# canyagmur/XPoint

Hardware: AMD Instinct MI355X
Metric: image-pairs/sec (detect+describe+match) 480x640 optical-thermal (higher is better)
Workload: dtype f32 (dense layers: f32 operands as 2 fp16 terms (operand error <= 2^-23, dropped cross term <= 2^-22: per product <= 2^-21 worst case, ~2^-25 typical), 3 fp16-MFMA partial products, f32 accumulate — GEMMs, implicit-GEMM convolutions and the fused block kernels alike; the deep-stage scan's dt project

## Files before the change

### xpoint_amd/csrc/elementwise.hip

```cpp
#include <stdlib.h>

#include <string>

#include <algorithm>

#include "glue_core.h"

namespace {

__global__ __launch_bounds__(256) void layernorm_kernel(const float* __restrict__ x, float* __restrict__ y,
                                                        const float* __restrict__ w, const float* __restrict__ b,
                                                        int64_t M, int C, float eps, int gelu) {
    const int lane = threadIdx.x & 63;
    const int64_t row = (int64_t)blockIdx.x * 4 + (threadIdx.x >> 6);
    if (row >= M) return;
    const float* xr = x + row * C;
    float v[16];
    float s = 0.f;
#pragma unroll
    for (int i = 0; i < 16; ++i) {
        const int c = lane + 64 * i;
        v[i] = (c < C) ? xr[c] : 0.f;
        s += v[i];
    }
// ... 13 lines not shown
        if (c < C) {
            float o = (v[i] - mean) * rstd * w[c] + b[c];
            if (gelu) o = xp_gelu(o);
            yr[c] = o;
        }
    }
}

template <int LPR, int NV, int RPG = 1, bool P32 = false>
__global__ __launch_bounds__(256) void layernorm_vec_kernel(const float* __restrict__ x, float* __restrict__ y,
                                                            const float* __restrict__ w, const float* __restrict__ b,
                                                            int64_t M, int C, float eps, int gelu) {
    constexpr int RPW = 64 / LPR;
    const int lane = threadIdx.x & 63, sub = lane % LPR;
    const int64_t row0 = ((int64_t)blockIdx.x * 4 + (threadIdx.x >> 6)) * (RPW * RPG) + lane / LPR;
    const int C4 = C >> 2;
    float4 v[RPG][NV];
    bool rok[RPG];
#pragma unroll
    for (int r = 0; r < RPG; ++r) {
        const int64_t row = row0 + r * RPW;
        rok[r] = row < M;
        const float4* xr = reinterpret_cast<const float4*>(x + (rok[r] ? row : 0) * C);
#pragma unroll
        for (int i = 0; i < NV; ++i) {
            const int c4 = sub + i * LPR;
            v[r][i] = (c4 < C4) ? xr[c4] : make_float4(0.f, 0.f, 0.f, 0.f);
        }
    }
#pragma unroll
    for (int r = 0; r < RPG; ++r) {
        float s = 0.f;
#pragma unroll
        for (int i = 0; i < NV; ++i) s += (v[r][i].x + v[r][i].y) + (v[r][i].z + v[r][i].w);
#pragma unroll
        for (int o = LPR / 2; o > 0; o >>= 1) s += __shfl_xor(s, o, 64);
        const float mean = s / (float)C;
        float q = 0.f;
#pragma unroll
        for (int i = 0; i < NV; ++i) {
            if (sub + i * LPR < C4) {
                const float dx = v[r][i].x - mean, dy = v[r][i].y - mean, dz = v[r][i].z - mean, dw = v[r][i].w - mean;
                q = fmaf(dx, dx, q); q = fmaf(dy, dy, q); q = fmaf(dz, dz, q); q = fmaf(dw, dw, q);
            }
        }
#pragma unroll
        for (int o = LPR / 2; o > 0; o >>= 1) q += __shfl_xor(q, o, 64);
        const float rstd = 1.f / sqrtf(q / (float)C + eps);
        if (!rok[r]) continue;
        float4* yr = reinterpret_cast<float4*>(y + (row0 + r * RPW) * C);
#pragma unroll
        for (int i = 0; i < NV; ++i) {
            const int c4 = sub + i * LPR;
            if (c4 < C4) {
                const float4 wv = reinterpret_cast<const float4*>(w)[c4], bv = reinterpret_cast<const float4*>(b)[c4];
                float4 o;
                o.x = (v[r][i].x - mean) * rstd * wv.x + bv.x; o.y = (v[r][i].y - mean) * rstd * wv.y + bv.y;
                o.z = (v[r][i].z - mean) * rstd * wv.z + bv.z; o.w = (v[r][i].w - mean) * rstd * wv.w + bv.w;
                if (gelu) { o.x = xp_gelu(o.x); o.y = xp_gelu(o.y); o.z = xp_gelu(o.z); o.w = xp_gelu(o.w); }
                if (P32) {
                    const xp_h4 hi = {(_Float16)o.x, (_Float16)o.y, (_Float16)o.z, (_Float16)o.w};
                    const xp_h4 lo = {(_Float16)(o.x - (float)hi[0]), (_Float16)(o.y - (float)hi[1]), (_Float16)(o.z - (float)hi[2]), (_Float16)(o.w - (float)hi[3])};
                    const int c = c4 * 4;
                    unsigned char* op = reinterpret_cast<unsigned char*>(y) + ((row0 + r * RPW) * (C >> 5) + (c >> 5)) * 128 + (c & 31) * 2;
                    *reinterpret_cast<xp_h4*>(op) = hi;
                    *reinterpret_cast<xp_h4*>(op + 64) = lo;
                } else
                yr[c4] = o;
            }
        }
    }
}

#ifndef XP_DW_PW
#define XP_DW_PW 4
#endif
#ifndef XP_DW_PH
#define XP_DW_PH 4
#endif
constexpr int DW_PW = XP_DW_PW, DW_PH = XP_DW_PH;
template <bool AMP>
__global__ __launch_bounds__(256) void dwconv3x3_silu_kernel(const float* __restrict__ x, const float* __restrict__ w,
                                                             float* __restrict__ y, int B, int H, int W, int C) {
    xp_dwconv3x3_silu_body<float, AMP, false, DW_PH, DW_PW>(x, w, y, nullptr, B, H, W, C, blockDim.x);
}

template <int CO, bool AMP>
__global__ __launch_bounds__(64) void stem_conv_ln_gelu_kernel(const float* __restrict__ img, const float* __restrict__ w9,
                                                               const float* __restrict__ bias, const float* __restrict__ lnw,
                                                               const float* __restrict__ lnb, float* __restrict__ y,
                                                               int B, int H, int W, float eps) {
    xp_stem_conv_ln_gelu_body<CO, float, AMP>(img, w9, bias, lnw, lnb, y, B, H, W, eps);
}

template <int CO>
__global__ __launch_bounds__(64) void stem_conv_kernel(const float* __restrict__ img, const float* __restrict__ w9, const float* __restrict__ bias,
                                                       float* __restrict__ y, int B, int H, int W) {
    xp_stem_conv_body<CO>(img, w9, bias, y, B, H, W);
}

__global__ __launch_bounds__(256) void depth_to_space_kernel(const float* __restrict__ x, float* __restrict__ y,
                                                             int B, int H, int W, int C, int bs, float limit, int* __restrict__ status) {
    const int Cq = C / (bs * bs);
    const int64_t total = (int64_t)B * H * W * C;
    const int64_t idx = (int64_t)blockIdx.x * blockDim.x + threadIdx.x;
    if (status) {
        const bool bad = idx < total && !(fabsf(x[idx]) < limit);
        if (__ballot(bad) != 0ull && (threadIdx.x & 63) == 0) atomicOr(status, XP_STATUS_ENC);
    }
    if (idx >= total) return;
    const int ch = (int)(idx % C);
    const int64_t pix = idx / C;
    const int w = (int)(pix % W), h = (int)((pix / W) % H);
    const int64_t n = pix / ((int64_t)W * H);
    const int blk = ch / Cq, c = ch - blk * Cq;
    const int i = blk / bs, j = blk - i * bs;
    y[((n * (H * bs) + (h * bs + i)) * (int64_t)(W * bs) + (w * bs + j)) * Cq + c] = x[idx];
}

__global__ __launch_bounds__(256) void depth_to_space_vec_kernel(const float4* __restrict__ x, float4* __restrict__ y,
                                                                 int B, int H, int W, int C4, int bs, float limit, int* __restrict__ status) {
    xp_depth_to_space_vec_body<float>(x, y, nullptr, B, H, W, C4, bs, limit, status, blockDim.x);
}

constexpr int SMX_CPW = 4;
__global__ __launch_bounds__(256) void softmax_shuffle_kernel(const float* __restrict__ logits, float* __restrict__ prob,
                                                              int B, int Hc, int Wc, int r, int ld, int mode, int* __restrict__ status) {
    const int lane = threadIdx.x & 63;
    const int64_t cell0 = ((int64_t)blockIdx.x * 4 + (threadIdx.x >> 6)) * SMX_CPW;
    const int64_t ncell = (int64_t)B * Hc * Wc;
    if (cell0 >= ncell) return;
    const int nch = r * r + 1;
    float v0[SMX_CPW], v1[SMX_CPW];
#pragma unroll
    for (int q = 0; q < SMX_CPW; ++q) {
        const int64_t cell = cell0 + q < ncell ? cell0 + q : ncell - 1;
        const float* lp = logits + cell * ld;
        v0[q] = (lane < nch) ? lp[lane] : -INFINITY;
        v1[q] = (lane + 64 < nch) ? lp[lane + 64] : -INFINITY;
    }
#pragma unroll
    for (int q = 0; q < SMX_CPW; ++q) {
        const int64_t cell = cell0 + q;
        if (cell >= ncell) break;
        float e0, e1, inv;
        if (mode == 0) {
            const float mx = xp_wave_max(fmaxf(v0[q], v1[q]));
            e0 = (lane < nch) ? expf(v0[q] - mx) : 0.f;
            e1 = (lane + 64 < nch) ? expf(v1[q] - mx) : 0.f;
            inv = 1.f / xp_wave_sum(e0 + e1);
            e0 *= inv; e1 *= inv;
            if (status && !(inv <= 1.f) && lane == 0) atomicOr(status, XP_STATUS_PROB);
        } else {
            e0 = (lane < nch) ? expf(v0[q]) : 0.f;
            e1 = (lane + 64 < nch) ? expf(v1[q]) : 0.f;
            const float den = xp_wave_sum(e0 + e1) + 0.00001f;
            e0 = e0 / den; e1 = e1 / den;
        }
        const int w = (int)(cell % Wc), h = (int)((cell / Wc) % Hc);
        const int64_t b = cell / ((int64_t)Wc * Hc);
        const int64_t Wf = (int64_t)Wc * r;
        for (int k = 0; k < 2; ++k) {
            const int ch = lane + 64 * k;
            if (ch < r * r) {
                const int i = ch / r, j = ch - i * r;
                prob[(b * Hc * r + (h * r + i)) * Wf + (w * r + j)] = k ? e1 : e0;
            }
        }
    }
}

// ... 82 lines not shown
    XP_CHECK_ARG(x && y && n >= 0, "xp_round_f16: bad args");
    XP_CHECK_ARG((((uintptr_t)x | (uintptr_t)y) & 15) == 0, "xp_round_f16: buffers must be 16-byte aligned");
    if (n == 0) return XP_OK;
    XpProfScope prof("round_f16", (hipStream_t)stream, 0.0, 8.0 * n);
    hipLaunchKernelGGL(round_f16_kernel, dim3(xp_cdiv(n, 1024)), dim3(256), 0, (hipStream_t)stream, x, y, n);
    XP_LAUNCH_CHECK();
    return XP_OK;
}

static int layernorm_impl(const float* x, float* y, const float* w, const float* b, int64_t rows, int C, float eps, int gelu, void* stream);
extern "C" int xp_layernorm(const float* x, float* y, const float* w, const float* b, int64_t rows, int C, float eps,
                            int gelu, void* stream) {
    if (xp_amp_value()) {
        XP_CHECK_ARG(gelu == 0, "xp_layernorm: the fused GELU has no mixed-precision form (the LayerNorm -> GELU boundary would not be rounded); use xp_stem_conv_ln_gelu or gelu = 0");
        XP_CHECK_ARG(C % 4 == 0 && ((uintptr_t)y & 15) == 0, "xp_layernorm: mixed-precision mode needs C %% 4 == 0 and a 16-byte aligned output (C = %d)", C);
    }
    const int rc = layernorm_impl(x, y, w, b, rows, C, eps, gelu, stream);
    if (rc == XP_OK && xp_amp_value() && rows > 0) return xp_round_f16(y, y, rows * C, stream);
    return rc;
}
static int layernorm_impl(const float* x, float* y, const float* w, const float* b, int64_t rows, int C, float eps,
                          int gelu, void* stream) {
    XP_CHECK_ARG(x && y && w && b, "xp_layernorm: null pointer");
    XP_CHECK_ARG(C > 0 && C <= 1024, "xp_layernorm: C must be in [1,1024] (got %d)", C);
    if (rows == 0) return XP_OK;
    XpProfScope prof(xp_prof_by_shape() ? ("layernorm_C" + std::to_string(C)).c_str() : "layernorm", (hipStream_t)stream, 8.0 * rows * C, 8.0 * rows * C);
    hipStream_t s = (hipStream_t)stream;
    const bool vec = (C % 4 == 0) && ((((uintptr_t)x | (uintptr_t)y | (uintptr_t)w | (uintptr_t)b) & 15) == 0);
    const int C4 = C / 4;
#define XP_LN_LAUNCH(LPR, NV) hipLaunchKernelGGL((layernorm_vec_kernel<LPR, NV, (NV == 1 ? 4 : 1)>), dim3(xp_cdiv(rows, 4 * (64 / LPR) * (NV == 1 ? 4 : 1))), dim3(256), 0, s, x, y, w, b, rows, C, eps, gelu)
    if (!vec) hipLaunchKernelGGL(layernorm_kernel, dim3(xp_cdiv(rows, 4)), dim3(256), 0, s, x, y, w, b, rows, C, eps, gelu);
    else if (C4 <= 4) XP_LN_LAUNCH(4, 1);
    else if (C4 <= 8) XP_LN_LAUNCH(8, 1);
    else if (C4 <= 16) XP_LN_LAUNCH(16, 1);
    else if (C4 <= 32) XP_LN_LAUNCH(32, 1);
    else if (C4 <= 64) XP_LN_LAUNCH(64, 1);
    else if (C4 <= 128) XP_LN_LAUNCH(64, 2);
    else if (C4 <= 192) XP_LN_LAUNCH(64, 3);
    else XP_LN_LAUNCH(64, 4);
#undef XP_LN_LAUNCH
    XP_LAUNCH_CHECK();
    return XP_OK;
}

extern "C" int xp_layernorm_p32(const float* x, void* y_p32, const float* w, const float* b, int64_t rows, int C, float eps, void* stream) {
    XP_CHECK_ARG(x && y_p32 && w && b, "xp_layernorm_p32: null pointer");
    XP_CHECK_ARG(C >= 32 && C <= 1024 && C % 32 == 0, "xp_layernorm_p32: C must be a multiple of 32 in [32, 1024] (got %d)", C);
    XP_CHECK_ARG((((uintptr_t)x | (uintptr_t)y_p32 | (uintptr_t)w | (uintptr_t)b) & 15) == 0, "xp_layernorm_p32: buffers must be 16-byte aligned");
    XP_CHECK_ARG(!xp_amp_value(), "xp_layernorm_p32: no mixed-precision form (the P32 image feeds the f32-grade ring GEMM only)");
    if (rows == 0) return XP_OK;
    XpProfScope prof("layernorm_p32", (hipStream_t)stream, 8.0 * rows * C, 8.0 * rows * C);
    hipStream_t s = (hipStream_t)stream;
    float* y = reinterpret_cast<float*>(y_p32);
    const int C4 = C / 4;
#define XP_LNP_LAUNCH(LPR, NV) hipLaunchKernelGGL((layernorm_vec_kernel<LPR, NV, (NV == 1 ? 4 : 1), true>), dim3(xp_cdiv(rows, 4 * (64 / LPR) * (NV == 1 ? 4 : 1))), dim3(256), 0, s, x, y, w, b, rows, C, eps, 0)
    if (C4 <= 8) XP_LNP_LAUNCH(8, 1);
    else if (C4 <= 16) XP_LNP_LAUNCH(16, 1);
    else if (C4 <= 32) XP_LNP_LAUNCH(32, 1);
    else if (C4 <= 64) XP_LNP_LAUNCH(64, 1);
    else if (C4 <= 128) XP_LNP_LAUNCH(64, 2);
    else if (C4 <= 192) XP_LNP_LAUNCH(64, 3);
    else XP_LNP_LAUNCH(64, 4);
#undef XP_LNP_LAUNCH
    XP_LAUNCH_CHECK();
    return XP_OK;
}

extern "C" int xp_dwconv3x3_silu(const float* x, const float* w9c, float* y, int batch, int H, int W, int C, void* stream) {
    XP_CHECK_ARG(x && w9c && y, "xp_dwconv3x3_silu: null pointer");
    XP_CHECK_ARG(C % 4 == 0, "xp_dwconv3x3_silu: C %% 4 != 0");
    const int64_t total = (int64_t)batch * ((H + DW_PH - 1) / DW_PH) * ((W + DW_PW - 1) / DW_PW) * (C / 4);
    XpProfScope prof("dwconv3x3_silu", (hipStream_t)stream, 22.0 * batch * H * W * C, 8.0 * batch * H * W * C);
    if (xp_amp_value()) hipLaunchKernelGGL(dwconv3x3_silu_kernel<true>, dim3(xp_cdiv(total, 256)), dim3(256), 0, (hipStream_t)stream, x, w9c, y, batch, H, W, C);
    else hipLaunchKernelGGL(dwconv3x3_silu_kernel<false>, dim3(xp_cdiv(total, 256)), dim3(256), 0, (hipStream_t)stream, x, w9c, y, batch, H, W, C);
    XP_LAUNCH_CHECK();
    return XP_OK;
}

extern "C" int xp_stem_conv_ln_gelu(const float* img, const float* w9co, const float* bias, const float* ln_w,
                                    const float* ln_b, float* y, int batch, int H, int W, int Co, float eps, void* stream) {
    XP_CHECK_ARG(img && w9co && bias && ln_w && ln_b && y, "xp_stem_conv_ln_gelu: null pointer");
    const int Ho = H / 2 + (H & 1), Wo = W / 2 + (W & 1);
    const int64_t total = (int64_t)batch * Ho * Wo;
    dim3 grid(xp_cdiv(total, 64)), block(64);
    hipStream_t s = (hipStream_t)stream;
    XpProfScope prof("stem_conv_ln_gelu", (hipStream_t)stream, (double)total * Co * 30.0, 4.0 * ((double)batch * H * W + (double)total * Co));
    const bool amp = xp_amp_value() != 0;
    if (Co == 48 && amp) hipLaunchKernelGGL((stem_conv_ln_gelu_kernel<48, true>), grid, block, 0, s, img, w9co, bias, ln_w, ln_b, y, batch, H, W, eps);
    else if (Co == 16 && amp) hipLaunchKernelGGL((stem_conv_ln_gelu_kernel<16, true>), grid, block, 0, s, img, w9co, bias, ln_w, ln_b, y, batch, H, W, eps);
    else if (Co == 48) hipLaunchKernelGGL((stem_conv_ln_gelu_kernel<48, false>), grid, block, 0, s, img, w9co, bias, ln_w, ln_b, y, batch, H, W, eps);
    else if (Co == 16) hipLaunchKernelGGL((stem_conv_ln_gelu_kernel<16, false>), grid, block, 0, s, img, w9co, bias, ln_w, ln_b, y, batch, H, W, eps);
    else { xp_set_error("xp_stem_conv_ln_gelu: Co must be 48 or 16 (EMBED_DIM 96 / 32), got %d", Co); return XP_ERR_ARG; }
    XP_LAUNCH_CHECK();
    return XP_OK;
}

extern "C" int xp_stem_conv(const float* img, const float* w9co, const float* bias, float* y, int batch, int H, int W, int Co, void* stream) {
    XP_CHECK_ARG(img && w9co && bias && y, "xp_stem_conv: null pointer");
    XP_CHECK_ARG(batch > 0 && H >= 1 && W >= 1, "xp_stem_conv: bad shape batch=%d H=%d W=%d", batch, H, W);
    const int Ho = H / 2 + (H & 1), Wo = W / 2 + (W & 1);
    const int64_t total = (int64_t)batch * Ho * Wo;
    dim3 grid(xp_cdiv(total, 64)), block(64);
    hipStream_t s = (hipStream_t)stream;
    XpProfScope prof("stem_conv", s, (double)total * Co * 18.0, 4.0 * ((double)batch * H * W + (double)total * Co));
    if (Co == 48) hipLaunchKernelGGL(stem_conv_kernel<48>, grid, block, 0, s, img, w9co, bias, y, batch, H, W);
    else if (Co == 16) hipLaunchKernelGGL(stem_conv_kernel<16>, grid, block, 0, s, img, w9co, bias, y, batch, H, W);
    else { xp_set_error("xp_stem_conv: Co must be 48 or 16 (EMBED_DIM 96 / 32), got %d", Co); return XP_ERR_ARG; }
    XP_LAUNCH_CHECK();
    return XP_OK;
}

int xp_depth_to_space_nhwc_st(const float* x, float* y, int batch, int H, int W, int C, int bs, float limit, int* status, void* stream) {
    XP_CHECK_ARG(x && y && C % (bs * bs) == 0, "xp_depth_to_space_nhwc: bad args");
    const int64_t total = (int64_t)batch * H * W * C;
    XpProfScope prof("depth_to_space", (hipStream_t)stream, 0.0, 8.0 * total);
    const bool vec = (C / (bs * bs)) % 4 == 0 && total < (1ll << 31) && ((((uintptr_t)x | (uintptr_t)y) & 15) == 0);
    if (vec) hipLaunchKernelGGL(depth_to_space_vec_kernel, dim3(xp_cdiv(total / 4, 256)), dim3(256), 0, (hipStream_t)stream, reinterpret_cast<const float4*>(x),
                                reinterpret_cast<float4*>(y), batch, H, W, C / 4, bs, limit, status);
    else hipLaunchKernelGGL(depth_to_space_kernel, dim3(xp_cdiv(total, 256)), dim3(256), 0, (hipStream_t)stream, x, y, batch, H, W, C, bs, limit, status);
    XP_LAUNCH_CHECK();
    return XP_OK;
}
extern "C" int xp_depth_to_space_nhwc(const float* x, float* y, int batch, int H, int W, int C, int bs, void* stream) {
    return xp_depth_to_space_nhwc_st(x, y, batch, H, W, C, bs, 0.f, nullptr, stream);
}

extern "C" int xp_softmax_shuffle(const float* logits, float* prob, int batch, int Hc, int Wc, int r, int ld, int mode, void* stream) {
    return xp_softmax_shuffle_st(logits, prob, batch, Hc, Wc, r, ld, mode, nullptr, stream);
}
int xp_softmax_shuffle_st(const float* logits, float* prob, int batch, int Hc, int Wc, int r, int ld, int mode, int* status, void* stream) {
    XP_CHECK_ARG(logits && prob, "xp_softmax_shuffle: null pointer");
    XP_CHECK_ARG(r * r + 1 <= 128 && ld >= r * r + 1, "xp_softmax_shuffle: r*r+1 must be <= 128 and <= ld");
    const int64_t cells = (int64_t)batch * Hc * Wc;
    XpProfScope prof("softmax_shuffle", (hipStream_t)stream, (double)cells * 4.0 * (r * r + 1), 4.0 * cells * (2.0 * r * r + 1));
    hipLaunchKernelGGL(softmax_shuffle_kernel, dim3(xp_cdiv(cells, 4 * SMX_CPW)), dim3(256), 0, (hipStream_t)stream, logits, prob, batch, Hc, Wc, r, ld, mode, status);
    XP_LAUNCH_CHECK();
    return XP_OK;
}

extern "C" int xp_l2norm_rows(const float* x, float* y, int64_t rows, int C, float eps, void* stream) {
    return xp_l2norm_rows_st(x, y, rows, C, eps, nullptr, stream);
}
int xp_l2norm_rows_st(const float* x, float* y, int64_t rows, int C, float eps, int* status, void* stream) {
    XP_CHECK_ARG(x && y, "xp_l2norm_rows: null pointer");
    if (rows == 0) return XP_OK;
    XpProfScope prof("l2norm_rows", (hipStream_t)stream, 3.0 * rows * C, 8.0 * rows * C);
    hipLaunchKernelGGL(l2norm_rows_kernel, dim3(xp_cdiv(rows, 4)), dim3(256), 0, (hipStream_t)stream, x, y, rows, C, eps, status);
    XP_LAUNCH_CHECK();
    return XP_OK;
}

extern "C" int xp_nhwc_to_nchw(const float* x, float* y, int batch, int HW, int C, void* stream) {
    XP_CHECK_ARG(x && y, "xp_nhwc_to_nchw: null pointer");
    dim3 grid(xp_cdiv(HW, 32), xp_cdiv(C, 32), batch);
    XpProfScope prof("nhwc_to_nchw", (hipStream_t)stream, 0.0, 8.0 * batch * HW * C);
    hipLaunchKernelGGL(nhwc_to_nchw_kernel, grid, dim3(256), 0, (hipStream_t)stream, x, y, HW, C);
    XP_LAUNCH_CHECK();
    return XP_OK;
}

__global__ __launch_bounds__(256) void stage_pair_batch_kernel(const float* __restrict__ a, const float* __restrict__ b, float* __restrict__ out,
                                                               const uint8_t* __restrict__ ma, const uint8_t* __restrict__ mb, uint8_t* __restrict__ mout,
                                                               int64_t n) {
    const int64_t stride = (int64_t)gridDim.x * blockDim.x, t0 = (int64_t)blockIdx.x * blockDim.x + threadIdx.x;
    const int64_t n4 = n >> 2;
    const bool al = ((reinterpret_cast<uintptr_t>(a) | reinterpret_cast<uintptr_t>(b) | reinterpret_cast<uintptr_t>(out) | (uintptr_t)(n * 4)) & 15) == 0;
    if (al) {
// ... 147 lines not shown
```

### xpoint_amd/csrc/elementwise_f16.hip

```cpp
#include <stdlib.h>

#include <string>

#include "glue_core.h"
#include "xpoint_hip.h"

namespace {

template <int CO>
__global__ __launch_bounds__(64) void stem_f16_kernel(const float* __restrict__ img, const float* __restrict__ w9, const float* __restrict__ bias,
                                                      const float* __restrict__ lnw, const float* __restrict__ lnb, _Float16* __restrict__ y,
                                                      int B, int H, int W, float eps) {
    xp_stem_conv_ln_gelu_body<CO, _Float16, true>(img, w9, bias, lnw, lnb, y, B, H, W, eps);
}

template <int LPR, int NV>
__global__ __launch_bounds__(256) void layernorm_f16_kernel(const _Float16* __restrict__ x, _Float16* __restrict__ y, const float* __restrict__ w,
                                                            const float* __restrict__ b, int64_t M, int C, float eps) {
    constexpr int RPW = 64 / LPR;
    const int lane = threadIdx.x & 63, sub = lane % LPR;
    const int64_t row = ((int64_t)blockIdx.x * 4 + (threadIdx.x >> 6)) * RPW + lane / LPR;
    const int C8 = C >> 3;
    const bool rok = row < M;
    const xp_h8* xr = reinterpret_cast<const xp_h8*>(x + (rok ? row : 0) * C);
    float v[NV][8];
    float s = 0.f;
#pragma unroll
    for (int i = 0; i < NV; ++i) {
        const int c8 = sub + i * LPR;
        xp_h8 t = {};
        if (c8 < C8) t = xr[c8];
#pragma unroll
        for (int e = 0; e < 8; ++e) { v[i][e] = (float)t[e]; }
        s += ((v[i][0] + v[i][1]) + (v[i][2] + v[i][3])) + ((v[i][4] + v[i][5]) + (v[i][6] + v[i][7]));
    }
#pragma unroll
    for (int o = LPR / 2; o > 0; o >>= 1) s += __shfl_xor(s, o, 64);
    const float mean = s / (float)C;
    float q = 0.f;
#pragma unroll
    for (int i = 0; i < NV; ++i)
        if (sub + i * LPR < C8) {
#pragma unroll
            for (int e = 0; e < 8; ++e) { const float d = v[i][e] - mean; q = fmaf(d, d, q); }
        }
#pragma unroll
    for (int o = LPR / 2; o > 0; o >>= 1) q += __shfl_xor(q, o, 64);
    const float rstd = 1.f / sqrtf(q / (float)C + eps);
    if (!rok) return;
    xp_h8* yr = reinterpret_cast<xp_h8*>(y + row * C);
#pragma unroll
    for (int i = 0; i < NV; ++i) {
        const int c8 = sub + i * LPR;
        if (c8 < C8) {
            const float4 w0 = reinterpret_cast<const float4*>(w)[2 * c8], w1 = reinterpret_cast<const float4*>(w)[2 * c8 + 1];
            const float4 b0 = reinterpret_cast<const float4*>(b)[2 * c8], b1 = reinterpret_cast<const float4*>(b)[2 * c8 + 1];
            const float wv[8] = {w0.x, w0.y, w0.z, w0.w, w1.x, w1.y, w1.z, w1.w}, bv[8] = {b0.x, b0.y, b0.z, b0.w, b1.x, b1.y, b1.z, b1.w};
            xp_h8 o;
#pragma unroll
            for (int e = 0; e < 8; ++e) o[e] = (_Float16)((v[i][e] - mean) * rstd * wv[e] + bv[e]);
            yr[c8] = o;
        }
    }
}

#ifndef XP_DWH_PW
#define XP_DWH_PW 4
#endif
#ifndef XP_DWH_PH
#define XP_DWH_PH 4
#endif
constexpr int DWH_PW = XP_DWH_PW, DWH_PH = XP_DWH_PH;
template <bool F32COPY>
__global__ __launch_bounds__(256) void dwconv3x3_silu_f16_kernel(const _Float16* __restrict__ x, const float* __restrict__ w, _Float16* __restrict__ y,
                                                                 float* __restrict__ y32, int B, int H, int W, int C) {
    xp_dwconv3x3_silu_body<_Float16, true, F32COPY, DWH_PH, DWH_PW>(x, w, y, y32, B, H, W, C, blockDim.x);
}

__global__ __launch_bounds__(256) void depth_to_space_f16_kernel(const xp_h4* __restrict__ x, float4* __restrict__ y32, xp_h4* __restrict__ y16,
                                                                 int B, int H, int W, int C4, int bs, int* __restrict__ status) {
    xp_depth_to_space_vec_body<_Float16>(x, y32, y16, B, H, W, C4, bs, INFINITY, status, blockDim.x);
}

}

extern "C" int xp_stem_conv_ln_gelu_f16(const float* img, const float* w9co, const float* bias, const float* ln_w, const float* ln_b, void* y,
                                        int batch, int H, int W, int CO, float eps, void* stream) {
    XP_CHECK_ARG(img && w9co && bias && ln_w && ln_b && y, "xp_stem_conv_ln_gelu_f16: null pointer");
    const int Ho = H / 2 + (H & 1), Wo = W / 2 + (W & 1);
    const int64_t total = (int64_t)batch * Ho * Wo;
    XpProfScope prof("stem_conv_ln_gelu_f16", (hipStream_t)stream, 0.0, 4.0 * batch * H * W + 2.0 * total * CO);
    const dim3 grid((unsigned)((total + 63) / 64));
    _Float16* yh = reinterpret_cast<_Float16*>(y);
    if (CO == 48) hipLaunchKernelGGL(stem_f16_kernel<48>, grid, dim3(64), 0, (hipStream_t)stream, img, w9co, bias, ln_w, ln_b, yh, batch, H, W, eps);
    else if (CO == 16) hipLaunchKernelGGL(stem_f16_kernel<16>, grid, dim3(64), 0, (hipStream_t)stream, img, w9co, bias, ln_w, ln_b, yh, batch, H, W, eps);
    else { xp_set_error("xp_stem_conv_ln_gelu_f16: CO must be 48 or 16 (got %d)", CO); return XP_ERR_ARG; }
    XP_LAUNCH_CHECK();
    return XP_OK;
}

extern "C" int xp_layernorm_f16(const void* x, void* y, const float* w, const float* b, int64_t rows, int C, float eps, void* stream) {
    XP_CHECK_ARG(x && y && w && b, "xp_layernorm_f16: null pointer");
    XP_CHECK_ARG(C > 0 && C % 8 == 0 && C <= 1024, "xp_layernorm_f16: C must be a multiple of 8 in [8, 1024] (got %d)", C);
    XP_CHECK_ARG((((uintptr_t)x | (uintptr_t)y | (uintptr_t)w | (uintptr_t)b) & 15) == 0, "xp_layernorm_f16: buffers must be 16-byte aligned");
    if (rows == 0) return XP_OK;
    XpProfScope prof(xp_prof_by_shape() ? ("layernorm_f16_C" + std::to_string(C)).c_str() : "layernorm_f16", (hipStream_t)stream, 8.0 * rows * C, 4.0 * rows * C);
    hipStream_t s = (hipStream_t)stream;
    const _Float16* xh = reinterpret_cast<const _Float16*>(x); _Float16* yh = reinterpret_cast<_Float16*>(y);
    const int C8 = C / 8;
#define XP_LNH(LPR, NV) hipLaunchKernelGGL((layernorm_f16_kernel<LPR, NV>), dim3(xp_cdiv(rows, 4 * (64 / LPR))), dim3(256), 0, s, xh, yh, w, b, rows, C, eps)
    if (C8 <= 4) XP_LNH(4, 1);
    else if (C8 <= 8) XP_LNH(8, 1);
    else if (C8 <= 16) XP_LNH(16, 1);
    else if (C8 <= 32) XP_LNH(32, 1);
    else if (C8 <= 64) XP_LNH(64, 1);
    else XP_LNH(64, 2);
#undef XP_LNH
    XP_LAUNCH_CHECK();
    return XP_OK;
}

extern "C" int xp_dwconv3x3_silu_f16(const void* x, const float* w9c, void* y, float* y_f32_copy, int batch, int H, int W, int C, void* stream) {
    XP_CHECK_ARG(x && w9c && y, "xp_dwconv3x3_silu_f16: null pointer");
    XP_CHECK_ARG(C % 4 == 0, "xp_dwconv3x3_silu_f16: C must be a multiple of 4 (got %d)", C);
    const int WG = (W + DWH_PW - 1) / DWH_PW, HG = (H + DWH_PH - 1) / DWH_PH;
    const int64_t total = (int64_t)batch * HG * WG * (C / 4);
    XpProfScope prof("dwconv3x3_silu_f16", (hipStream_t)stream, 0.0, (4.0 + (y_f32_copy ? 4.0 : 0.0)) * batch * H * W * C);
    const dim3 grid((unsigned)((total + 255) / 256));
    const _Float16* xh = reinterpret_cast<const _Float16*>(x); _Float16* yh = reinterpret_cast<_Float16*>(y);
    if (y_f32_copy) hipLaunchKernelGGL(dwconv3x3_silu_f16_kernel<true>, grid, dim3(256), 0, (hipStream_t)stream, xh, w9c, yh, y_f32_copy, batch, H, W, C);
    else hipLaunchKernelGGL(dwconv3x3_silu_f16_kernel<false>, grid, dim3(256), 0, (hipStream_t)stream, xh, w9c, yh, (float*)nullptr, batch, H, W, C);
    XP_LAUNCH_CHECK();
    return XP_OK;
}

extern "C" int xp_depth_to_space_nhwc_f16(const void* x, float* y_f32, void* y_f16, int batch, int H, int W, int C, int bs, int* status, void* stream) {
    XP_CHECK_ARG(x && y_f32 && y_f16, "xp_depth_to_space_nhwc_f16: null pointer");
    XP_CHECK_ARG(bs > 0 && C % (bs * bs) == 0 && (C / (bs * bs)) % 4 == 0, "xp_depth_to_space_nhwc_f16: C / bs^2 must be a multiple of 4");
    const int64_t n4 = (int64_t)batch * H * W * (C / 4);
    XP_CHECK_ARG(n4 < (1ll << 31), "xp_depth_to_space_nhwc_f16: tensor too large");
    XpProfScope prof("depth_to_space_f16", (hipStream_t)stream, 0.0, 8.0 * 4.0 * n4);
    hipLaunchKernelGGL(depth_to_space_f16_kernel, dim3((unsigned)((n4 + 255) / 256)), dim3(256), 0, (hipStream_t)stream, reinterpret_cast<const xp_h4*>(x),
                       reinterpret_cast<float4*>(y_f32), reinterpret_cast<xp_h4*>(y_f16), batch, H, W, C / 4, bs, status);
    XP_LAUNCH_CHECK();
    return XP_OK;
}
```

### xpoint_amd/csrc/glue_core.h

```cpp
#pragma once
#include "xp_common.h"

typedef _Float16 xp_h4 __attribute__((ext_vector_type(4)));
typedef _Float16 xp_h8 __attribute__((ext_vector_type(8)));

template <typename T> struct XpGlueVec;
template <> struct XpGlueVec<float> { typedef float4 v4; };
template <> struct XpGlueVec<_Float16> { typedef xp_h4 v4; };
template <typename T> constexpr bool xp_glue_half = sizeof(T) == 2;

__device__ __forceinline__ float4 xp_glue_f4(const float4 v) { return v; }
__device__ __forceinline__ float4 xp_glue_f4(const xp_h4 v) { return make_float4((float)v[0], (float)v[1], (float)v[2], (float)v[3]); }
__device__ __forceinline__ float4 xp_r16(const float4 v) { return make_float4(xp_r16(v.x), xp_r16(v.y), xp_r16(v.z), xp_r16(v.w)); }

template <typename T, bool R16, bool F32COPY, int PH, int PW>
__device__ __forceinline__ void xp_dwconv3x3_silu_body(const T* __restrict__ x, const float* __restrict__ w, T* __restrict__ y, float* __restrict__ y32,
                                                       int B, int H, int W, int C, unsigned nthr) {
    static_assert(R16 || !xp_glue_half<T>, "fp16 storage rounds at every store");
    typedef typename XpGlueVec<T>::v4 V;
    const int C4 = C >> 2;
    const int WG = (W + PW - 1) / PW, HG = (H + PH - 1) / PH;
    const int64_t total = (int64_t)B * HG * WG * C4;
    const unsigned nb = gridDim.x, xcd = blockIdx.x & 7, slot = blockIdx.x >> 3, q = nb >> 3, r = nb & 7;
    const unsigned blk = (xcd < r ? xcd * (q + 1) : r * (q + 1) + (xcd - r) * q) + slot;
    const int64_t idx = (int64_t)blk * nthr + threadIdx.x;
    if (idx >= total) return;
    const int c4 = (int)(idx % C4);
    const int64_t g = idx / C4;
    const int w0 = (int)(g % WG) * PW;
    const int h0 = (int)((g / WG) % HG) * PH;
    const int64_t b = g / ((int64_t)WG * HG);
    const V* xv = reinterpret_cast<const V*>(x);
    float4 wt[9];
#pragma unroll
    for (int t = 0; t < 9; ++t) wt[t] = reinterpret_cast<const float4*>(w)[t * C4 + c4];
    float4 acc[PH][PW];
#pragma unroll
    for (int rr = 0; rr < PH; ++rr)
#pragma unroll
        for (int p = 0; p < PW; ++p) acc[rr][p] = make_float4(0.f, 0.f, 0.f, 0.f);
#pragma unroll
    for (int ir = 0; ir < PH + 2; ++ir) {
        const int ih = h0 + ir - 1;
        if (ih < 0 || ih >= H) continue;
        float4 col[PW + 2];
#pragma unroll
        for (int cx = 0; cx < PW + 2; ++cx) {
            const int iw = w0 + cx - 1;
            if constexpr (xp_glue_half<T>) {
                V t = {};
                if (iw >= 0 && iw < W) t = xv[((b * H + ih) * W + iw) * C4 + c4];
                col[cx] = xp_glue_f4(t);
            } else {
                col[cx] = (iw >= 0 && iw < W) ? xv[((b * H + ih) * W + iw) * C4 + c4] : make_float4(0.f, 0.f, 0.f, 0.f);
            }
        }
#pragma unroll
        for (int rr = 0; rr < PH; ++rr) {
            const int kh = ir - rr;
            if (kh < 0 || kh > 2) continue;
#pragma unroll
            for (int p = 0; p < PW; ++p)
#pragma unroll
                for (int kw = 0; kw < 3; ++kw) {
                    const int iw = w0 + p + kw - 1;
                    if (iw < 0 || iw >= W) continue;
                    const float4 xin = col[p + kw], wv = wt[kh * 3 + kw];
                    acc[rr][p].x = fmaf(xin.x, wv.x, acc[rr][p].x); acc[rr][p].y = fmaf(xin.y, wv.y, acc[rr][p].y);
                    acc[rr][p].z = fmaf(xin.z, wv.z, acc[rr][p].z); acc[rr][p].w = fmaf(xin.w, wv.w, acc[rr][p].w);
                }
        }
    }
#pragma unroll
    for (int rr = 0; rr < PH; ++rr) {
        if (h0 + rr >= H) break;
#pragma unroll
        for (int p = 0; p < PW; ++p) {
            if (w0 + p >= W) break;
            float4 o = acc[rr][p];
            if (R16) o = xp_r16(o);
            o.x = xp_silu(o.x); o.y = xp_silu(o.y); o.z = xp_silu(o.z); o.w = xp_silu(o.w);
            if (R16) o = xp_r16(o);
            const int64_t oi = ((b * H + h0 + rr) * W + w0 + p) * C4 + c4;
            if constexpr (xp_glue_half<T>) reinterpret_cast<V*>(y)[oi] = V{(_Float16)o.x, (_Float16)o.y, (_Float16)o.z, (_Float16)o.w};
            else reinterpret_cast<V*>(y)[oi] = o;
            if (F32COPY) reinterpret_cast<float4*>(y32)[oi] = o;
        }
    }
}

template <int CO, bool R16>
__device__ __forceinline__ float xp_stem_conv_pixel(const float* __restrict__ img, const float* s_w, int64_t b, int oh, int ow, int H, int W, float (&acc)[CO]) {
    float xin[9];
#pragma unroll
    for (int kh = 0; kh < 3; ++kh)
#pragma unroll
        for (int kw = 0; kw < 3; ++kw) {
            const int ih = oh * 2 + kh - 1, iw = ow * 2 + kw - 1;
            xin[kh * 3 + kw] = (ih >= 0 && ih < H && iw >= 0 && iw < W) ? img[(b * H + ih) * W + iw] : 0.f;
            if (R16) xin[kh * 3 + kw] = xp_r16(xin[kh * 3 + kw]);
        }
    float s = 0.f;
#pragma unroll
    for (int c = 0; c < CO; ++c) {
        float a = 0.f;
#pragma unroll
        for (int t = 0; t < 9; ++t) a = fmaf(xin[t], s_w[t * CO + c], a);
        a += s_w[9 * CO + c];
        if (R16) a = xp_r16(a);
        acc[c] = a; s += a;
    }
    return s;
}

template <int CO, typename T, bool R16>
__device__ __forceinline__ void xp_stem_conv_ln_gelu_body(const float* __restrict__ img, const float* __restrict__ w9, const float* __restrict__ bias,
                                                          const float* __restrict__ lnw, const float* __restrict__ lnb, T* __restrict__ y,
                                                          int B, int H, int W, float eps) {
    static_assert(R16 || !xp_glue_half<T>, "fp16 storage rounds at every store");
    constexpr int LDO = CO + (xp_glue_half<T> ? 2 : 1);
    __shared__ float s_w[12 * CO];
    __shared__ T s_o[64 * LDO];
    for (int i = threadIdx.x; i < 9 * CO; i += 64) s_w[i] = w9[i];
    for (int i = threadIdx.x; i < CO; i += 64) { s_w[9 * CO + i] = bias[i]; s_w[10 * CO + i] = lnw[i]; s_w[11 * CO + i] = lnb[i]; }
    __syncthreads();
    const int Ho = H / 2 + (H & 1), Wo = W / 2 + (W & 1);
    const int64_t total = (int64_t)B * Ho * Wo;
    const int64_t p0 = (int64_t)blockIdx.x * 64;
    const int64_t pix = p0 + threadIdx.x;
    if (pix < total) {
        const int ow = (int)(pix % Wo), oh = (int)((pix / Wo) % Ho);
        const int64_t b = pix / ((int64_t)Wo * Ho);
        float acc[CO];
        const float s = xp_stem_conv_pixel<CO, R16>(img, s_w, b, oh, ow, H, W, acc);
        const float mean = s / (float)CO;
        float q = 0.f;
#pragma unroll
        for (int c = 0; c < CO; ++c) { const float d = acc[c] - mean; q = fmaf(d, d, q); }
        const float rstd = 1.f / sqrtf(q / (float)CO + eps);
#pragma unroll
        for (int c = 0; c < CO; ++c) {
            float v = (acc[c] - mean) * rstd * s_w[10 * CO + c] + s_w[11 * CO + c];
            if (R16) v = xp_r16(v);
            v = xp_gelu_fast(v);
            if (R16) v = xp_r16(v);
            s_o[threadIdx.x * LDO + c] = (T)v;
        }
    }
    __syncthreads();
    const int64_t nvalid = (total - p0 < 64) ? (total - p0) : 64;
    for (int i = threadIdx.x; i < nvalid * CO; i += 64) {
        const int pl = i / CO, c = i - pl * CO;
        y[(p0 + pl) * CO + c] = s_o[pl * LDO + c];
    }
}

template <int CO>
__device__ __forceinline__ void xp_stem_conv_body(const float* __restrict__ img, const float* __restrict__ w9, const float* __restrict__ bias,
                                                  float* __restrict__ y, int B, int H, int W) {
    constexpr int LDO = CO + 1;
    __shared__ float s_w[10 * CO];
    __shared__ float s_o[64 * LDO];
    for (int i = threadIdx.x; i < 9 * CO; i += 64) s_w[i] = w9[i];
    for (int i = threadIdx.x; i < CO; i += 64) s_w[9 * CO + i] = bias[i];
    __syncthreads();
    const int Ho = H / 2 + (H & 1), Wo = W / 2 + (W & 1);
    const int64_t total = (int64_t)B * Ho * Wo;
    const int64_t p0 = (int64_t)blockIdx.x * 64;
    const int64_t pix = p0 + threadIdx.x;
    if (pix < total) {
        const int ow = (int)(pix % Wo), oh = (int)((pix / Wo) % Ho);
        const int64_t b = pix / ((int64_t)Wo * Ho);
        float acc[CO];
        (void)xp_stem_conv_pixel<CO, false>(img, s_w, b, oh, ow, H, W, acc);
#pragma unroll
        for (int c = 0; c < CO; ++c) s_o[threadIdx.x * LDO + c] = acc[c];
    }
    __syncthreads();
    const int64_t nvalid = (total - p0 < 64) ? (total - p0) : 64;
    for (int i = threadIdx.x; i < nvalid * CO; i += 64) {
        const int pl = i / CO, c = i - pl * CO;
        y[(p0 + pl) * CO + c] = s_o[pl * LDO + c];
    }
}

template <typename T>
__device__ __forceinline__ void xp_depth_to_space_vec_body(const typename XpGlueVec<T>::v4* __restrict__ x, float4* __restrict__ y32,
                                                           typename XpGlueVec<T>::v4* __restrict__ y16, int B, int H, int W, int C4, int bs,
                                                           float limit, int* __restrict__ status, unsigned nthr) {
    typedef typename XpGlueVec<T>::v4 V;
    const int Cq4 = C4 / (bs * bs);
    const unsigned total = (unsigned)B * H * W * C4;
    const unsigned idx = blockIdx.x * nthr + threadIdx.x;
    V v;
    if constexpr (xp_glue_half<T>) { v = V{}; if (idx < total) v = x[idx]; }
    else v = idx < total ? x[idx] : make_float4(0.f, 0.f, 0.f, 0.f);
    const float4 f = xp_glue_f4(v);
    if (status) {
        const bool bad = !(fabsf(f.x) < limit) || !(fabsf(f.y) < limit) || !(fabsf(f.z) < limit) || !(fabsf(f.w) < limit);
        if (__ballot(bad && idx < total) != 0ull && (threadIdx.x & 63) == 0) atomicOr(status, XP_STATUS_ENC);
    }
    if (idx >= total) return;
    const unsigned ch = idx % (unsigned)C4, pix = idx / (unsigned)C4;
    const unsigned w = pix % (unsigned)W, hn = pix / (unsigned)W, h = hn % (unsigned)H, n = hn / (unsigned)H;
    const unsigned blk = ch / (unsigned)Cq4, c = ch - blk * Cq4;
    const unsigned i = blk / (unsigned)bs, j = blk - i * bs;
    const unsigned o = ((n * (H * bs) + (h * bs + i)) * (unsigned)(W * bs) + (w * bs + j)) * Cq4 + c;
    y32[o] = f;
    if constexpr (xp_glue_half<T>) y16[o] = v;
}
```

Baseline: 1849.

## Add 32-bit buffer-load interior path for fp16 dwconv and widen stem kernel

The fp16 depthwise 3x3+SiLU kernel gains a 32-bit-index variant. When a whole wavefront is interior, it uses raw buffer loads and stores with scalar offsets and no bounds checks. The stem conv+LN+GELU kernel moves from 64 to 256 threads per block. It reads weights directly from global memory instead of staging them in LDS, and stages output as 16-byte chunks for vectorised coalesced stores. The aim is to cut index arithmetic, branch overhead and narrow stores in these memory-bound glue kernels, at the cost of more template variants and reliance on the wavefront-uniform interior check.

```diff
diff --git a/xpoint_amd/csrc/elementwise.hip b/xpoint_amd/csrc/elementwise.hip
--- a/xpoint_amd/csrc/elementwise.hip
+++ b/xpoint_amd/csrc/elementwise.hip
@@ -119,11 +119,11 @@
 template <bool AMP>
 __global__ __launch_bounds__(256) void dwconv3x3_silu_kernel(const float* __restrict__ x, const float* __restrict__ w,
                                                              float* __restrict__ y, int B, int H, int W, int C) {
-    xp_dwconv3x3_silu_body<float, AMP, false, DW_PH, DW_PW>(x, w, y, nullptr, B, H, W, C, blockDim.x);
+    xp_dwconv3x3_silu_body<float, AMP, false, DW_PH, DW_PW, false>(x, w, y, nullptr, B, H, W, C, blockDim.x);
 }
 
 template <int CO, bool AMP>
-__global__ __launch_bounds__(64) void stem_conv_ln_gelu_kernel(const float* __restrict__ img, const float* __restrict__ w9,
+__global__ __launch_bounds__(XP_STEM_NT) void stem_conv_ln_gelu_kernel(const float* __restrict__ img, const float* __restrict__ w9,
                                                                const float* __restrict__ bias, const float* __restrict__ lnw,
                                                                const float* __restrict__ lnb, float* __restrict__ y,
                                                                int B, int H, int W, float eps) {
@@ -372,7 +372,7 @@
     XP_CHECK_ARG(img && w9co && bias && ln_w && ln_b && y, "xp_stem_conv_ln_gelu: null pointer");
     const int Ho = H / 2 + (H & 1), Wo = W / 2 + (W & 1);
     const int64_t total = (int64_t)batch * Ho * Wo;
-    dim3 grid(xp_cdiv(total, 64)), block(64);
+    dim3 grid(xp_cdiv(total, XP_STEM_NT)), block(XP_STEM_NT);
     hipStream_t s = (hipStream_t)stream;
     XpProfScope prof("stem_conv_ln_gelu", (hipStream_t)stream, (double)total * Co * 30.0, 4.0 * ((double)batch * H * W + (double)total * Co));
     const bool amp = xp_amp_value() != 0;
diff --git a/xpoint_amd/csrc/elementwise_f16.hip b/xpoint_amd/csrc/elementwise_f16.hip
--- a/xpoint_amd/csrc/elementwise_f16.hip
+++ b/xpoint_amd/csrc/elementwise_f16.hip
@@ -8,7 +8,7 @@
 namespace {
 
 template <int CO>
-__global__ __launch_bounds__(64) void stem_f16_kernel(const float* __restrict__ img, const float* __restrict__ w9, const float* __restrict__ bias,
+__global__ __launch_bounds__(XP_STEM_NT) void stem_f16_kernel(const float* __restrict__ img, const float* __restrict__ w9, const float* __restrict__ bias,
                                                       const float* __restrict__ lnw, const float* __restrict__ lnb, _Float16* __restrict__ y,
                                                       int B, int H, int W, float eps) {
     xp_stem_conv_ln_gelu_body<CO, _Float16, true>(img, w9, bias, lnw, lnb, y, B, H, W, eps);
@@ -71,10 +71,10 @@
 #define XP_DWH_PH 4
 #endif
 constexpr int DWH_PW = XP_DWH_PW, DWH_PH = XP_DWH_PH;
-template <bool F32COPY>
+template <bool F32COPY, bool IDX32>
 __global__ __launch_bounds__(256) void dwconv3x3_silu_f16_kernel(const _Float16* __restrict__ x, const float* __restrict__ w, _Float16* __restrict__ y,
                                                                  float* __restrict__ y32, int B, int H, int W, int C) {
-    xp_dwconv3x3_silu_body<_Float16, true, F32COPY, DWH_PH, DWH_PW>(x, w, y, y32, B, H, W, C, blockDim.x);
+    xp_dwconv3x3_silu_body<_Float16, true, F32COPY, DWH_PH, DWH_PW, IDX32>(x, w, y, y32, B, H, W, C, blockDim.x);
 }
 
 __global__ __launch_bounds__(256) void depth_to_space_f16_kernel(const xp_h4* __restrict__ x, float4* __restrict__ y32, xp_h4* __restrict__ y16,
@@ -90,10 +90,10 @@
     const int Ho = H / 2 + (H & 1), Wo = W / 2 + (W & 1);
     const int64_t total = (int64_t)batch * Ho * Wo;
     XpProfScope prof("stem_conv_ln_gelu_f16", (hipStream_t)stream, 0.0, 4.0 * batch * H * W + 2.0 * total * CO);
-    const dim3 grid((unsigned)((total + 63) / 64));
+    const dim3 grid((unsigned)((total + XP_STEM_NT - 1) / XP_STEM_NT));
     _Float16* yh = reinterpret_cast<_Float16*>(y);
-    if (CO == 48) hipLaunchKernelGGL(stem_f16_kernel<48>, grid, dim3(64), 0, (hipStream_t)stream, img, w9co, bias, ln_w, ln_b, yh, batch, H, W, eps);
-    else if (CO == 16) hipLaunchKernelGGL(stem_f16_kernel<16>, grid, dim3(64), 0, (hipStream_t)stream, img, w9co, bias, ln_w, ln_b, yh, batch, H, W, eps);
+    if (CO == 48) hipLaunchKernelGGL(stem_f16_kernel<48>, grid, dim3(XP_STEM_NT), 0, (hipStream_t)stream, img, w9co, bias, ln_w, ln_b, yh, batch, H, W, eps);
+    else if (CO == 16) hipLaunchKernelGGL(stem_f16_kernel<16>, grid, dim3(XP_STEM_NT), 0, (hipStream_t)stream, img, w9co, bias, ln_w, ln_b, yh, batch, H, W, eps);
     else { xp_set_error("xp_stem_conv_ln_gelu_f16: CO must be 48 or 16 (got %d)", CO); return XP_ERR_ARG; }
     XP_LAUNCH_CHECK();
     return XP_OK;
@@ -128,8 +128,13 @@
     XpProfScope prof("dwconv3x3_silu_f16", (hipStream_t)stream, 0.0, (4.0 + (y_f32_copy ? 4.0 : 0.0)) * batch * H * W * C);
     const dim3 grid((unsigned)((total + 255) / 256));
     const _Float16* xh = reinterpret_cast<const _Float16*>(x); _Float16* yh = reinterpret_cast<_Float16*>(y);
-    if (y_f32_copy) hipLaunchKernelGGL(dwconv3x3_silu_f16_kernel<true>, grid, dim3(256), 0, (hipStream_t)stream, xh, w9c, yh, y_f32_copy, batch, H, W, C);
-    else hipLaunchKernelGGL(dwconv3x3_silu_f16_kernel<false>, grid, dim3(256), 0, (hipStream_t)stream, xh, w9c, yh, (float*)nullptr, batch, H, W, C);
+    const bool i32 = xp_glue_idx32(batch, H, W, C);
+#define XP_DWH(COPY, I32) hipLaunchKernelGGL((dwconv3x3_silu_f16_kernel<COPY, I32>), grid, dim3(256), 0, (hipStream_t)stream, xh, w9c, yh, y_f32_copy, batch, H, W, C)
+    if (y_f32_copy && i32) XP_DWH(true, true);
+    else if (y_f32_copy) XP_DWH(true, false);
+    else if (i32) XP_DWH(false, true);
+    else XP_DWH(false, false);
+#undef XP_DWH
     XP_LAUNCH_CHECK();
     return XP_OK;
 }
diff --git a/xpoint_amd/csrc/glue_core.h b/xpoint_amd/csrc/glue_core.h
--- a/xpoint_amd/csrc/glue_core.h
+++ b/xpoint_amd/csrc/glue_core.h
@@ -1,4 +1,7 @@
 #pragma once
+#include <type_traits>
+
+#include "glue_idx.h"
 #include "xp_common.h"
 
 typedef _Float16 xp_h4 __attribute__((ext_vector_type(4)));
@@ -11,25 +14,56 @@
 
 __device__ __forceinline__ float4 xp_glue_f4(const float4 v) { return v; }
 __device__ __forceinline__ float4 xp_glue_f4(const xp_h4 v) { return make_float4((float)v[0], (float)v[1], (float)v[2], (float)v[3]); }
+typedef unsigned xp_u4 __attribute__((ext_vector_type(4)));
+typedef unsigned xp_u2 __attribute__((ext_vector_type(2)));
+__device__ __forceinline__ __amdgpu_buffer_rsrc_t xp_glue_rsrc(const void* p, unsigned bytes) {
+    return __builtin_amdgcn_make_buffer_rsrc(const_cast<void*>(p), 0, (int)bytes, 0x00020000);
+}
+__device__ __forceinline__ void xp_glue_buf_load(float4& v, __amdgpu_buffer_rsrc_t r, unsigned voff, unsigned soff) {
+    v = __builtin_bit_cast(float4, __builtin_amdgcn_raw_buffer_load_b128(r, voff, soff, 0));
+}
+__device__ __forceinline__ void xp_glue_buf_load(xp_h4& v, __amdgpu_buffer_rsrc_t r, unsigned voff, unsigned soff) {
+    v = __builtin_bit_cast(xp_h4, __builtin_amdgcn_raw_buffer_load_b64(r, voff, soff, 0));
+}
+__device__ __forceinline__ void xp_glue_buf_store(const float4 v, __amdgpu_buffer_rsrc_t r, unsigned voff) {
+    __builtin_amdgcn_raw_buffer_store_b128(__builtin_bit_cast(xp_u4, v), r, voff, 0, 0);
+}
+__device__ __forceinline__ void xp_glue_buf_store(const xp_h4 v, __amdgpu_buffer_rsrc_t r, unsigned voff) {
+    __builtin_amdgcn_raw_buffer_store_b64(__builtin_bit_cast(xp_u2, v), r, voff, 0, 0);
+}
 __device__ __forceinline__ float4 xp_r16(const float4 v) { return make_float4(xp_r16(v.x), xp_r16(v.y), xp_r16(v.z), xp_r16(v.w)); }
 
-template <typename T, bool R16, bool F32COPY, int PH, int PW>
+template <bool R16>
+__device__ __forceinline__ float4 xp_dwconv_finish(float4 o) {
+    if (R16) o = xp_r16(o);
+    o.x = xp_silu(o.x); o.y = xp_silu(o.y); o.z = xp_silu(o.z); o.w = xp_silu(o.w);
+    if (R16) o = xp_r16(o);
+    return o;
+}
+template <typename T>
+__device__ __forceinline__ typename XpGlueVec<T>::v4 xp_glue_pack(const float4 o) {
+    if constexpr (xp_glue_half<T>) return xp_h4{(_Float16)o.x, (_Float16)o.y, (_Float16)o.z, (_Float16)o.w};
+    else return o;
+}
+
+template <typename T, bool R16, bool F32COPY, int PH, int PW, bool IDX32>
 __device__ __forceinline__ void xp_dwconv3x3_silu_body(const T* __restrict__ x, const float* __restrict__ w, T* __restrict__ y, float* __restrict__ y32,
                                                        int B, int H, int W, int C, unsigned nthr) {
     static_assert(R16 || !xp_glue_half<T>, "fp16 storage rounds at every store");
     typedef typename XpGlueVec<T>::v4 V;
+    typedef typename std::conditional<IDX32, unsigned, int64_t>::type I;
     const int C4 = C >> 2;
     const int WG = (W + PW - 1) / PW, HG = (H + PH - 1) / PH;
-    const int64_t total = (int64_t)B * HG * WG * C4;
+    const I total = (I)B * HG * WG * C4;
     const unsigned nb = gridDim.x, xcd = blockIdx.x & 7, slot = blockIdx.x >> 3, q = nb >> 3, r = nb & 7;
     const unsigned blk = (xcd < r ? xcd * (q + 1) : r * (q + 1) + (xcd - r) * q) + slot;
-    const int64_t idx = (int64_t)blk * nthr + threadIdx.x;
+    const I idx = (I)blk * nthr + threadIdx.x;
     if (idx >= total) return;
     const int c4 = (int)(idx % C4);
-    const int64_t g = idx / C4;
+    const I g = idx / C4;
     const int w0 = (int)(g % WG) * PW;
     const int h0 = (int)((g / WG) % HG) * PH;
-    const int64_t b = g / ((int64_t)WG * HG);
+    const I b = g / ((I)WG * HG);
     const V* xv = reinterpret_cast<const V*>(x);
     float4 wt[9];
 #pragma unroll
@@ -39,6 +73,46 @@
     for (int rr = 0; rr < PH; ++rr)
 #pragma unroll
         for (int p = 0; p < PW; ++p) acc[rr][p] = make_float4(0.f, 0.f, 0.f, 0.f);
+    if constexpr (IDX32) {
+        const bool inner = h0 >= 1 && h0 + PH < H && w0 >= 1 && w0 + PW < W;
+        if (__ballot(!inner) == 0ull) {
+            const unsigned rs = (unsigned)W * C4;
+            const unsigned first = ((b * H + (h0 - 1)) * W + (w0 - 1)) * C4 + c4;
+            const unsigned off = first * (unsigned)sizeof(V), off32 = first * (unsigned)sizeof(float4);
+            const unsigned n4 = (unsigned)B * H * W * C4;
+            const __amdgpu_buffer_rsrc_t xr = xp_glue_rsrc(x, n4 * (unsigned)sizeof(V)), yr = xp_glue_rsrc(y, n4 * (unsigned)sizeof(V)),
+                                         yr32 = xp_glue_rsrc(y32, F32COPY ? n4 * (unsigned)sizeof(float4) : 0u);
+#pragma unroll
+            for (int ir = 0; ir < PH + 2; ++ir) {
+                float4 col[PW + 2];
+#pragma unroll
+                for (int cx = 0; cx < PW + 2; ++cx) { V t; xp_glue_buf_load(t, xr, off, (ir * rs + cx * (unsigned)C4) * (unsigned)sizeof(V)); col[cx] = xp_glue_f4(t); }
+#pragma unroll
+                for (int rr = 0; rr < PH; ++rr) {
+                    const int kh = ir - rr;
+                    if (kh < 0 || kh > 2) continue;
+#pragma unroll
+                    for (int p = 0; p < PW; ++p)
+#pragma unroll
+                        for (int kw = 0; kw < 3; ++kw) {
+                            const float4 xin = col[p + kw], wv = wt[kh * 3 + kw];
+                            acc[rr][p].x = fmaf(xin.x, wv.x, acc[rr][p].x); acc[rr][p].y = fmaf(xin.y, wv.y, acc[rr][p].y);
+                            acc[rr][p].z = fmaf(xin.z, wv.z, acc[rr][p].z); acc[rr][p].w = fmaf(xin.w, wv.w, acc[rr][p].w);
+                        }
+                }
+                if (ir >= 2) {
+#pragma unroll
+                    for (int p = 0; p < PW; ++p) {
+                        const unsigned o = (ir - 1) * rs + (p + 1) * (unsigned)C4;
+                        const float4 v = xp_dwconv_finish<R16>(acc[ir - 2][p]);
+                        xp_glue_buf_store(xp_glue_pack<T>(v), yr, off + o * (unsigned)sizeof(V));
+                        if (F32COPY) xp_glue_buf_store(v, yr32, off32 + o * (unsigned)sizeof(float4));
+                    }
+                }
+            }
+            return;
+        }
+    }
 #pragma unroll
     for (int ir = 0; ir < PH + 2; ++ir) {
         const int ih = h0 + ir - 1;
@@ -77,20 +151,17 @@
 #pragma unroll
         for (int p = 0; p < PW; ++p) {
             if (w0 + p >= W) break;
-            float4 o = acc[rr][p];
-            if (R16) o = xp_r16(o);
-            o.x = xp_silu(o.x); o.y = xp_silu(o.y); o.z = xp_silu(o.z); o.w = xp_silu(o.w);
-            if (R16) o = xp_r16(o);
-            const int64_t oi = ((b * H + h0 + rr) * W + w0 + p) * C4 + c4;
-            if constexpr (xp_glue_half<T>) reinterpret_cast<V*>(y)[oi] = V{(_Float16)o.x, (_Float16)o.y, (_Float16)o.z, (_Float16)o.w};
-            else reinterpret_cast<V*>(y)[oi] = o;
-            if (F32COPY) reinterpret_cast<float4*>(y32)[oi] = o;
-        }
-    }
-}
-
-template <int CO, bool R16>
-__device__ __forceinline__ float xp_stem_conv_pixel(const float* __restrict__ img, const float* s_w, int64_t b, int oh, int ow, int H, int W, float (&acc)[CO]) {
+            const I oi = ((b * H + h0 + rr) * W + w0 + p) * C4 + c4;
+            const float4 v = xp_dwconv_finish<R16>(acc[rr][p]);
+            reinterpret_cast<V*>(y)[oi] = xp_glue_pack<T>(v);
+            if (F32COPY) reinterpret_cast<float4*>(y32)[oi] = v;
+        }
+    }
+}
+
+template <int CO, bool R16, bool SW>
+__device__ __forceinline__ float xp_stem_conv_pixel(const float* __restrict__ img, const float* __restrict__ w, const float* __restrict__ bias, int64_t b, int oh,
+                                                    int ow, int H, int W, float (&acc)[CO]) {
     float xin[9];
 #pragma unroll
     for (int kh = 0; kh < 3; ++kh)
@@ -103,55 +174,73 @@
     float s = 0.f;
 #pragma unroll
     for (int c = 0; c < CO; ++c) {
+        if (SW && c % 4 == 0) asm volatile("" ::: "memory");
         float a = 0.f;
 #pragma unroll
-        for (int t = 0; t < 9; ++t) a = fmaf(xin[t], s_w[t * CO + c], a);
-        a += s_w[9 * CO + c];
+        for (int t = 0; t < 9; ++t) a = fmaf(xin[t], w[t * CO + c], a);
+        a += bias[c];
         if (R16) a = xp_r16(a);
         acc[c] = a; s += a;
     }
     return s;
 }
+
+constexpr int XP_STEM_NT = 256;
+template <typename T> struct XpGlueChunk;
+template <> struct XpGlueChunk<float> { typedef float type __attribute__((ext_vector_type(4))); };
+template <> struct XpGlueChunk<_Float16> { typedef xp_h8 type; };
 
 template <int CO, typename T, bool R16>
 __device__ __forceinline__ void xp_stem_conv_ln_gelu_body(const float* __restrict__ img, const float* __restrict__ w9, const float* __restrict__ bias,
                                                           const float* __restrict__ lnw, const float* __restrict__ lnb, T* __restrict__ y,
                                                           int B, int H, int W, float eps) {
     static_assert(R16 || !xp_glue_half<T>, "fp16 storage rounds at every store");
-    constexpr int LDO = CO + (xp_glue_half<T> ? 2 : 1);
-    __shared__ float s_w[12 * CO];
-    __shared__ T s_o[64 * LDO];
-    for (int i = threadIdx.x; i < 9 * CO; i += 64) s_w[i] = w9[i];
-    for (int i = threadIdx.x; i < CO; i += 64) { s_w[9 * CO + i] = bias[i]; s_w[10 * CO + i] = lnw[i]; s_w[11 * CO + i] = lnb[i]; }
-    __syncthreads();
+    typedef typename XpGlueChunk<T>::type Chunk;
+    constexpr int CH = 16 / (int)sizeof(T), CPR = CO / CH, LDC = CPR + 1;
+    static_assert(CO % CH == 0, "a pixel is a whole number of 16-byte chunks");
+    __shared__ Chunk s_o[XP_STEM_NT * LDC];
     const int Ho = H / 2 + (H & 1), Wo = W / 2 + (W & 1);
     const int64_t total = (int64_t)B * Ho * Wo;
-    const int64_t p0 = (int64_t)blockIdx.x * 64;
+    const int64_t p0 = (int64_t)blockIdx.x * XP_STEM_NT;
     const int64_t pix = p0 + threadIdx.x;
     if (pix < total) {
         const int ow = (int)(pix % Wo), oh = (int)((pix / Wo) % Ho);
         const int64_t b = pix / ((int64_t)Wo * Ho);
         float acc[CO];
-        const float s = xp_stem_conv_pixel<CO, R16>(img, s_w, b, oh, ow, H, W, acc);
+        const float s = xp_stem_conv_pixel<CO, R16, true>(img, w9, bias, b, oh, ow, H, W, acc);
         const float mean = s / (float)CO;
         float q = 0.f;
 #pragma unroll
         for (int c = 0; c < CO; ++c) { const float d = acc[c] - mean; q = fmaf(d, d, q); }
         const float rstd = 1.f / sqrtf(q / (float)CO + eps);
 #pragma unroll
-        for (int c = 0; c < CO; ++c) {
-            float v = (acc[c] - mean) * rstd * s_w[10 * CO + c] + s_w[11 * CO + c];
-            if (R16) v = xp_r16(v);
-            v = xp_gelu_fast(v);
-            if (R16) v = xp_r16(v);
-            s_o[threadIdx.x * LDO + c] = (T)v;
+        for (int cc = 0; cc < CPR; ++cc) {
+            asm volatile("" ::: "memory");
+            Chunk o;
+#pragma unroll
+            for (int e = 0; e < CH; ++e) {
+                const int c = cc * CH + e;
+                float v = (acc[c] - mean) * rstd * lnw[c] + lnb[c];
+                if (R16) v = xp_r16(v);
+                v = xp_gelu_fast(v);
+                if (R16) v = xp_r16(v);
+                o[e] = (T)v;
+            }
+            s_o[threadIdx.x * LDC + cc] = o;
         }
     }
     __syncthreads();
-    const int64_t nvalid = (total - p0 < 64) ? (total - p0) : 64;
-    for (int i = threadIdx.x; i < nvalid * CO; i += 64) {
-        const int pl = i / CO, c = i - pl * CO;
-        y[(p0 + pl) * CO + c] = s_o[pl * LDO + c];
+    const int nvalid = (total - p0 < XP_STEM_NT) ? (int)(total - p0) : XP_STEM_NT;
+    T* yt = y + p0 * CO;
+    if ((reinterpret_cast<uintptr_t>(y) & 15) == 0) {
+#pragma unroll
+        for (int k = 0; k < CPR; ++k) {
+            const int j = threadIdx.x + k * XP_STEM_NT;
+            if (j < nvalid * CPR) { const int pl = j / CPR; reinterpret_cast<Chunk*>(yt)[j] = s_o[pl * LDC + (j - pl * CPR)]; }
+        }
+    } else {
+        const T* s_e = reinterpret_cast<const T*>(s_o);
+        for (int i = threadIdx.x; i < nvalid * CO; i += XP_STEM_NT) { const int pl = i / CO; yt[i] = s_e[pl * (LDC * CH) + (i - pl * CO)]; }
     }
 }
 
@@ -172,7 +261,7 @@
         const int ow = (int)(pix % Wo), oh = (int)((pix / Wo) % Ho);
         const int64_t b = pix / ((int64_t)Wo * Ho);
         float acc[CO];
-        (void)xp_stem_conv_pixel<CO, false>(img, s_w, b, oh, ow, H, W, acc);
+        (void)xp_stem_conv_pixel<CO, false, false>(img, s_w, s_w + 9 * CO, b, oh, ow, H, W, acc);
 #pragma unroll
         for (int c = 0; c < CO; ++c) s_o[threadIdx.x * LDO + c] = acc[c];
     }
diff --git a/xpoint_amd/csrc/glue_idx.h b/xpoint_amd/csrc/glue_idx.h
--- /dev/null
+++ b/xpoint_amd/csrc/glue_idx.h
@@ -0,0 +1,11 @@
+#pragma once
+#include <stdint.h>
+
+inline bool xp_glue_idx32(int B, int H, int W, int C) {
+    const int64_t lim = int64_t(1) << 30;
+    int64_t n = (int64_t)B * H;
+    if (n >= lim) return false;
+    n *= W;
+    if (n >= lim) return false;
+    return n * C < lim;
+}
```

After: 1860, median of 6. About the same (+0.6%).
